# jinlinyi/PerspectiveFields

Hardware: NVIDIA H100
Metric: images/sec at 640x480 (Paramnet-360Cities-edina), H100 vs ref CPU (higher is better)
Workload: dtype f32 via 3x bf16 split MMA, fp32 accumulate

## Files before the change

perspectivefields_b200/csrc/gemm_tma.cuh:

```cuda
#pragma once
#include <cuda.h>

#include "tc_ptx.cuh"

namespace pf {

constexpr int MODE_GEMM = 0, MODE_HALO = 1;
constexpr int kTmaThreads = 384;
constexpr int kHaloBytes = 180 * 128;

struct TmaGemmParams {
  int M;
  int B, H, W;
  int Cin;
  int N, K;
  int a_c0, a_gc;
  int c_split, a2_c0;
  int groups;
  int b_row0;
  const float* bias; int bias_mode, bias_gstride;
  int act; const float* gamma;
  const float* res;  int ldr, r_coff, r_gcoff, res_relu;
  const float* res2; int ldr2, r2_coff, r2_gcoff;
  float* C; int ldc, c_coff, c_gcoff;
  __nv_bfloat16* Shi; __nv_bfloat16* Slo; int lds, s_coff, s_gcoff, split_relu;
  const float* pred_w; const float* pred_b; float* pred_out; int pred_nc, pred_mode;
  int phase4;
};

template <int BN, int MODE, int KB, bool PP = false, int NP = 3> struct TmaCfg {
  static_assert(KB == 32 || KB == 64, "KB");
  static_assert(BN % 32 == 0 && BN <= 256, "BN");
  static_assert(!PP || MODE == MODE_GEMM, "the ping-pong schedule is a GEMM-mode schedule");
  static_assert(NP == 1 || NP == 3, "NP");
  static constexpr int kPlanes = NP == 3 ? 2 : 1;
  static constexpr int kTileM = PP ? 64 : 128;
  static constexpr int kBPlane = BN * KB * 2;
  static constexpr int kAPlane = kTileM * KB * 2;
  static constexpr int kStage = (MODE == MODE_GEMM ? kPlanes * kAPlane : 0) + kPlanes * kBPlane;
  static constexpr int kABuf = kPlanes * kHtPlaneBytes;
  static constexpr int kAccPitch = 68;
  static constexpr int kAccStage = 2 * 64 * kAccPitch * 4;
  static constexpr int kBudget = 225 * 1024 - kAccStage - (MODE == MODE_HALO ? 2 * kABuf : 0);
  static constexpr int kStagesRaw = kBudget / kStage;
  static constexpr int kStages = kStagesRaw > 16 ? 16 : kStagesRaw;
  static constexpr int kSmemBytes = (MODE == MODE_HALO ? 2 * kABuf : 0) + kStages * kStage + kAccStage + 512 + 1024;
  static_assert(kStages >= 2, "ring too shallow");
  static_assert(kSmemBytes <= 227 * 1024, "shared memory per block");
};

__device__ __forceinline__ void mbar_expect_tx(uint32_t bar, uint32_t bytes) {
  asm volatile("mbarrier.arrive.expect_tx.shared::cta.b64 _, [%0], %1;\n" ::"r"(bar), "r"(bytes) : "memory");
}
__device__ __forceinline__ void tma_load_2d(uint32_t dst, const CUtensorMap* map, uint32_t bar, int c0, int c1) {
  asm volatile("cp.async.bulk.tensor.2d.shared::cluster.global.mbarrier::complete_tx::bytes [%0], [%1, {%3, %4}], [%2];\n"
               ::"r"(dst), "l"(reinterpret_cast<uint64_t>(map)), "r"(bar), "r"(c0), "r"(c1) : "memory");
}
__device__ __forceinline__ void tma_load_4d(uint32_t dst, const CUtensorMap* map, uint32_t bar, int c0, int c1, int c2, int c3) {
  asm volatile("cp.async.bulk.tensor.4d.shared::cluster.global.mbarrier::complete_tx::bytes [%0], [%1, {%3, %4, %5, %6}], [%2];\n"
               ::"r"(dst), "l"(reinterpret_cast<uint64_t>(map)), "r"(bar), "r"(c0), "r"(c1), "r"(c2), "r"(c3) : "memory");
}
__device__ __forceinline__ void tma_prefetch_desc(const CUtensorMap* map) {
  asm volatile("prefetch.tensormap [%0];\n" ::"l"(reinterpret_cast<uint64_t>(map)) : "memory");
}

struct TmaMaps {
  CUtensorMap a_hi, a_lo, a2_hi, a2_lo, b_hi, b_lo;
};

template <int BN, int MODE, int KB, bool PP = false, int NP = 3>
__global__ void __launch_bounds__(kTmaThreads, 1) gemm_tma_kernel(const __grid_constant__ TmaMaps maps, const TmaGemmParams p, int tiles_x, int tiles_y) {
  using Cfg = TmaCfg<BN, MODE, KB, PP, NP>;
  constexpr bool kLo = NP == 3;
  constexpr int NS = Cfg::kStages;
  constexpr int SPC = 9 * (64 / KB);
  constexpr int kConsumerWarps = PP ? 4 : 8;
  extern __shared__ unsigned char smem_dyn[];
  const uint32_t raw = smem_u32(smem_dyn);
  const uint32_t sbase = (raw + 1023u) & ~1023u;
  unsigned char* sm = smem_dyn + (sbase - raw);
  const uint32_t a_base = sbase;
  const uint32_t ring = sbase + (MODE == MODE_HALO ? 2 * Cfg::kABuf : 0);
  const uint32_t acc_base = ring + NS * Cfg::kStage;
  const uint32_t bars = acc_base + Cfg::kAccStage;
  auto full_b = [&](int s) { return bars + 8u * s; };
  auto empty_b = [&](int s) { return bars + 8u * (NS + s); };
  auto full_a = [&](int i) { return bars + 8u * (2 * NS + i); };
  auto empty_a = [&](int i) { return bars + 8u * (2 * NS + 2 + i); };
  auto order_b = [&](int w) { return bars + 8u * (2 * NS + 4 + w); };

  const int tid = threadIdx.x, lane = tid & 31, warp = tid >> 5;
  const int n_tiles = cdiv(p.N, BN);
  const int m_tiles = MODE == MODE_GEMM ? cdiv(p.M, Cfg::kTileM) : p.B * tiles_x * tiles_y;
  const int total_tiles = m_tiles * n_tiles * p.groups;
  const int nchunks = MODE == MODE_HALO ? p.Cin / 64 : 0;
  const int nk = MODE == MODE_GEMM ? p.K / KB : nchunks * SPC;
  const bool b_resident = MODE == MODE_HALO && nchunks == 1 && SPC <= NS;

  if (tid == 0) {
    tma_prefetch_desc(&maps.a_hi); tma_prefetch_desc(&maps.b_hi);
    if (kLo) { tma_prefetch_desc(&maps.a_lo); tma_prefetch_desc(&maps.b_lo); }
    for (int s = 0; s < NS; ++s) { mbar_init(full_b(s), 1); mbar_init(empty_b(s), kConsumerWarps); }
    for (int i = 0; i < 2; ++i) { mbar_init(full_a(i), 1); mbar_init(empty_a(i), kConsumerWarps); mbar_init(order_b(i), 4); }
    fence_mbar_init();
  }
  __syncthreads();
  pdl_wait();
  pdl_launch();

  auto decode = [&](int tile, int& mt, int& g, int& n0) {
    n0 = (tile % n_tiles) * BN;
    tile /= n_tiles;
    g = tile % p.groups;
    mt = tile / p.groups;
  };

  if (warp < 4) {
    asm volatile("setmaxnreg.dec.sync.aligned.u32 40;\n");
    if (warp == 0 && lane == 0) {
      int it = 0;
      for (int tile = blockIdx.x; tile < total_tiles; tile += gridDim.x) {
        int mt, g, n0;
        decode(tile, mt, g, n0);
        const int brow = p.b_row0 + g * p.N + n0;
        if (b_resident && it > 0) break;
        for (int kc = 0; kc < nk; ++kc, ++it) {
          const int s = it % NS;
          mbar_wait(empty_b(s), ((it / NS) & 1) ^ 1);
          mbar_expect_tx(full_b(s), Cfg::kStage);
          const uint32_t st = ring + s * Cfg::kStage;
          int kcol;
          if (MODE == MODE_GEMM) {
            kcol = kc * KB;
            tma_load_2d(st, &maps.a_hi, full_b(s), p.a_c0 + g * p.a_gc + kcol, mt * Cfg::kTileM);
            if (kLo) tma_load_2d(st + Cfg::kAPlane, &maps.a_lo, full_b(s), p.a_c0 + g * p.a_gc + kcol, mt * Cfg::kTileM);
          } else {
            const int c = kc / SPC, u = kc - c * SPC;
            kcol = KB == 32 ? (u >> 1) * p.Cin + c * 64 + (u & 1) * 32 : u * p.Cin + c * 64;
          }
          const uint32_t bdst = st + (MODE == MODE_GEMM ? Cfg::kPlanes * Cfg::kAPlane : 0);
          tma_load_2d(bdst, &maps.b_hi, full_b(s), kcol, brow);
          if (kLo) tma_load_2d(bdst + Cfg::kBPlane, &maps.b_lo, full_b(s), kcol, brow);
        }
      }
    } else if (MODE == MODE_HALO && warp == 1 && lane == 0) {
      int ita = 0;
      for (int tile = blockIdx.x; tile < total_tiles; tile += gridDim.x) {
        int mt, g, n0;
        decode(tile, mt, g, n0);
        const int tx = mt % tiles_x, ty = (mt / tiles_x) % tiles_y, bimg = mt / (tiles_x * tiles_y);
        for (int c = 0; c < nchunks; ++c, ++ita) {
          const int buf = ita & 1;
          mbar_wait(empty_a(buf), ((ita >> 1) & 1) ^ 1);
          mbar_expect_tx(full_a(buf), Cfg::kPlanes * kHaloBytes);
          const uint32_t dst = a_base + buf * Cfg::kABuf;
          const int ci = c * 64;
          if (p.c_split > 0 && ci >= p.c_split) {
            tma_load_4d(dst, &maps.a2_hi, full_a(buf), p.a2_c0 + ci - p.c_split, tx * kHtTileW - 1, ty * kHtTileH - 1, bimg);
            if (kLo) tma_load_4d(dst + kHtPlaneBytes, &maps.a2_lo, full_a(buf), p.a2_c0 + ci - p.c_split, tx * kHtTileW - 1, ty * kHtTileH - 1, bimg);
          } else {
            tma_load_4d(dst, &maps.a_hi, full_a(buf), p.a_c0 + g * p.a_gc + ci, tx * kHtTileW - 1, ty * kHtTileH - 1, bimg);
            if (kLo) tma_load_4d(dst + kHtPlaneBytes, &maps.a_lo, full_a(buf), p.a_c0 + g * p.a_gc + ci, tx * kHtTileW - 1, ty * kHtTileH - 1, bimg);
          }
        }
      }
    }
    return;
  }

  asm volatile("setmaxnreg.inc.sync.aligned.u32 232;\n");
  const int wg = (warp >> 2) - 1;
  const int wt = tid & 127;
  float* stage = reinterpret_cast<float*>(sm + (acc_base - sbase)) + wg * 64 * Cfg::kAccPitch;
  const int erow = wt & 63, eh = wt >> 6;
  const int r = PP ? erow : wg * 64 + erow;
  constexpr int kTileStep = PP ? 2 : 1;
  float acc[BN / 2];
  int it = 0, ita = 0;
  for (int tl = PP ? wg : 0, tile = blockIdx.x + tl * gridDim.x; tile < total_tiles; tile += kTileStep * gridDim.x, tl += kTileStep) {
    int mt, g, n0;
    decode(tile, mt, g, n0);
    if (PP) {
      it = tl * nk;
      if (tl > 0) mbar_wait(order_b(wg ^ 1), ((tl - 1) >> 1) & 1);
    }
    int prev_s = -1, prev_buf = -1;
    fence_regs(acc);
    for (int kc = 0; kc < nk; ++kc, ++it) {
      const int s = it % NS;
      uint32_t a_hi, a_lo;
      bool chunk_end = false;
      int buf = 0;
      if (MODE == MODE_HALO) {
        const int c = kc / SPC, u = kc - c * SPC;
        const int tap = KB == 32 ? (u >> 1) : u, ky = tap / 3, kx = tap - ky * 3;
        buf = ita & 1;
        if (u == 0) mbar_wait(full_a(buf), (ita >> 1) & 1);
        a_hi = a_base + buf * Cfg::kABuf + ((ky + 8 * wg) * kHtHaloW + kx) * 128 + (KB == 32 ? (u & 1) * 64 : 0);
        a_lo = a_hi + kHtPlaneBytes;
        chunk_end = u == SPC - 1;
      } else {
        a_hi = ring + s * Cfg::kStage + (PP ? 0 : wg * 64 * KB * 2);
        a_lo = a_hi + Cfg::kAPlane;
      }
      const int sb = b_resident ? kc : s;
      if (!b_resident || tl == 0) mbar_wait(full_b(sb), b_resident ? 0 : ((it / NS) & 1));
      const uint32_t b_hi = ring + sb * Cfg::kStage + (MODE == MODE_GEMM ? Cfg::kPlanes * Cfg::kAPlane : 0);
      const uint64_t dah = MODE == MODE_HALO ? ht_a_desc(a_hi) : wgmma_tile_desc<KB>(a_hi);
      const uint64_t dbh = wgmma_tile_desc<KB>(b_hi);
      wgmma_fence();
      if (kLo) {
        const uint64_t dal = MODE == MODE_HALO ? ht_a_desc(a_lo) : wgmma_tile_desc<KB>(a_lo);
        const uint64_t dbl = wgmma_tile_desc<KB>(b_hi + Cfg::kBPlane);
#pragma unroll
        for (int kk = 0; kk < KB / 16; ++kk) {
          const uint32_t first = (kc | kk) ? 1u : 0u;
          wgmma_bf16<BN>(acc, dal + 2 * kk, dbh + 2 * kk, first);
          wgmma_bf16<BN>(acc, dah + 2 * kk, dbl + 2 * kk, 1u);
          wgmma_bf16<BN>(acc, dah + 2 * kk, dbh + 2 * kk, 1u);
        }
      } else {
#pragma unroll
        for (int kk = 0; kk < KB / 16; ++kk) wgmma_bf16<BN>(acc, dah + 2 * kk, dbh + 2 * kk, (kc | kk) ? 1u : 0u);
      }
      wgmma_commit();
      wgmma_wait<1>();
      if (lane == 0 && prev_s >= 0) {
        if (!b_resident) mbar_arrive(empty_b(prev_s));
        if (MODE == MODE_HALO && prev_buf >= 0) mbar_arrive(empty_a(prev_buf));
      }
      prev_s = s;
      prev_buf = chunk_end ? buf : -1;
      if (MODE == MODE_HALO && chunk_end) ++ita;
    }
    if (PP && lane == 0) mbar_arrive(order_b(wg));
    wgmma_wait<0>();
    fence_regs(acc);
    if (lane == 0 && prev_s >= 0) {
      if (!b_resident) mbar_arrive(empty_b(prev_s));
      if (MODE == MODE_HALO && prev_buf >= 0) mbar_arrive(empty_a(prev_buf));
    }

    long long m;
    bool valid;
    int cls_off = 0;
    int bimg = 0, oy = 0, ox = 0, oy0 = 0, ox0 = 0;
    if (MODE == MODE_GEMM) {
      m = (long long)mt * Cfg::kTileM + r;
      valid = m < p.M;
    } else {
      const int tx = mt % tiles_x, ty = (mt / tiles_x) % tiles_y;
      bimg = mt / (tiles_x * tiles_y);
      oy0 = ty * kHtTileH; ox0 = tx * kHtTileW;
      oy = oy0 + (r >> 3); ox = ox0 + (r & 7);
      valid = oy < p.H && ox < p.W;
      m = ((long long)bimg * p.H + oy) * p.W + ox;
      if (p.bias_mode == 2) {
        const int ry = oy == 0 ? 0 : (oy == p.H - 1 ? 2 : 1);
        const int rx = ox == 0 ? 0 : (ox == p.W - 1 ? 2 : 1);
        cls_off = (ry * 3 + rx) * p.N;
      }
    }
    const float* __restrict__ bias = p.bias ? p.bias + (long long)g * p.bias_gstride : nullptr;
    auto stage_row = [&](int rr, long long& mr) -> bool {
      if (MODE == MODE_GEMM) {
        mr = (long long)mt * Cfg::kTileM + (PP ? 0 : wg * 64) + rr;
        return mr < p.M;
      }
      const int rt = wg * 64 + rr, py = oy0 + (rt >> 3), px = ox0 + (rt & 7);
      mr = ((long long)bimg * p.H + py) * p.W + px;
      return py < p.H && px < p.W;
    };
    const int frow = (wt >> 5) * 16 + (lane >> 2), fcol = 2 * (lane & 3);
#pragma unroll
    for (int rd = 0; rd < (BN + 63) / 64; ++rd) {
      named_bar_sync(1 + wg, 128);
#pragma unroll
      for (int jb = 0; jb < 8; ++jb) {
        const int cb = rd * 8 + jb;
        if (cb < BN / 8) {
          float* d0 = stage + frow * Cfg::kAccPitch + jb * 8 + fcol;
          *reinterpret_cast<float2*>(d0) = make_float2(acc[4 * cb], acc[4 * cb + 1]);
          *reinterpret_cast<float2*>(d0 + 8 * Cfg::kAccPitch) = make_float2(acc[4 * cb + 2], acc[4 * cb + 3]);
        }
      }
      named_bar_sync(1 + wg, 128);
      const int ch = 2 * rd + eh;
      const bool own = ch < BN / 32;
      const bool ph4 = MODE == MODE_HALO && BN == 128 && p.phase4;
      const bool staged_split = p.Shi && !ph4;
      const int nb = n0 + ch * 32;
      const bool chunk_ok = own && nb < p.N;
      const bool live = valid && chunk_ok;
      const float* srow = stage + erow * Cfg::kAccPitch + eh * 32;
      float o[32];
      if (own) {
#pragma unroll
        for (int j = 0; j < 32; j += 4) {
          const float4 t = *reinterpret_cast<const float4*>(srow + j);
          o[j] = t.x; o[j + 1] = t.y; o[j + 2] = t.z; o[j + 3] = t.w;
        }
      }
      if (live) {
        if (p.bias_mode) {
#pragma unroll
          for (int j = 0; j < 32; j += 4) {
            const float4 bv = __ldg(reinterpret_cast<const float4*>(bias + cls_off + nb + j));
            o[j] += bv.x; o[j + 1] += bv.y; o[j + 2] += bv.z; o[j + 3] += bv.w;
          }
        }
        if (p.act == 1) {
#pragma unroll
          for (int j = 0; j < 32; ++j) o[j] = fmaxf(o[j], 0.f);
        } else if (p.act == 2) {
#pragma unroll
          for (int j = 0; j < 32; ++j) o[j] = gelu_erf(o[j]);
        }
        if (p.gamma) {
#pragma unroll
          for (int j = 0; j < 32; j += 4) {
            const float4 gv = __ldg(reinterpret_cast<const float4*>(p.gamma + nb + j));
            o[j] *= gv.x; o[j + 1] *= gv.y; o[j + 2] *= gv.z; o[j + 3] *= gv.w;
          }
        }
      }
      auto stage_in = [&](const float* src, int ld, int coff) {
        named_bar_sync(1 + wg, 128);
        float4 v[8];
#pragma unroll
        for (int t = 0; t < 8; ++t) {
          const int i = wt + 128 * t, col = rd * 64 + (i & 15) * 4;
          long long mr;
          v[t] = make_float4(0.f, 0.f, 0.f, 0.f);
          if (col < BN && n0 + col < p.N && stage_row(i >> 4, mr)) v[t] = *reinterpret_cast<const float4*>(src + mr * ld + coff + n0 + col);
        }
#pragma unroll
        for (int t = 0; t < 8; ++t) {
          const int i = wt + 128 * t;
          *reinterpret_cast<float4*>(stage + (i >> 4) * Cfg::kAccPitch + (i & 15) * 4) = v[t];
        }
        named_bar_sync(1 + wg, 128);
      };
      if (p.res) {
        stage_in(p.res, p.ldr, p.r_coff + g * p.r_gcoff);
        if (live) {
#pragma unroll
          for (int j = 0; j < 32; j += 4) {
            float4 rv = *reinterpret_cast<const float4*>(srow + j);
            if (p.res_relu) { rv.x = fmaxf(rv.x, 0.f); rv.y = fmaxf(rv.y, 0.f); rv.z = fmaxf(rv.z, 0.f); rv.w = fmaxf(rv.w, 0.f); }
            o[j] += rv.x; o[j + 1] += rv.y; o[j + 2] += rv.z; o[j + 3] += rv.w;
          }
        }
      }
      if (p.res2) {
        stage_in(p.res2, p.ldr2, p.r2_coff + g * p.r2_gcoff);
        if (live) {
#pragma unroll
          for (int j = 0; j < 32; j += 4) {
            const float4 rv = *reinterpret_cast<const float4*>(srow + j);
            o[j] += rv.x; o[j + 1] += rv.y; o[j + 2] += rv.z; o[j + 3] += rv.w;
          }
        }
      }
      const long long mo = ph4 ? ((long long)bimg * 2 * p.H + 2 * oy + (ch >> 1)) * (2 * p.W) + 2 * ox + (ch & 1) : m;
      if (MODE == MODE_HALO && (BN == 32 || BN == 128) && p.pred_w && live) {
        float v0 = __ldg(p.pred_b), v1 = p.pred_nc > 1 ? __ldg(p.pred_b + 1) : 0.f;
#pragma unroll
        for (int j = 0; j < 32; j += 4) {
          const float4 w0 = __ldg(reinterpret_cast<const float4*>(p.pred_w + j));
          v0 = fmaf(o[j], w0.x, v0); v0 = fmaf(o[j + 1], w0.y, v0); v0 = fmaf(o[j + 2], w0.z, v0); v0 = fmaf(o[j + 3], w0.w, v0);
          if (p.pred_nc > 1) {
            const float4 w1 = __ldg(reinterpret_cast<const float4*>(p.pred_w + 32 + j));
            v1 = fmaf(o[j], w1.x, v1); v1 = fmaf(o[j + 1], w1.y, v1); v1 = fmaf(o[j + 2], w1.z, v1); v1 = fmaf(o[j + 3], w1.w, v1);
          }
        }
        const long long HWl = (long long)p.H * p.W * (ph4 ? 4 : 1);
        const long long bi = mo / HWl, pix = mo - bi * HWl;
        float* po = p.pred_out + bi * p.pred_nc * HWl + pix;
        if (p.pred_mode == 1) {
          const float nrm = fmaxf(sqrtf(v0 * v0 + v1 * v1), 1e-12f);
          po[0] = v0 / nrm; po[HWl] = v1 / nrm;
        } else {
          po[0] = fminf(fmaxf(v0, -1.f), 1.f);
        }
      }
      if (ph4 && chunk_ok && (p.C || p.Shi)) {
        const bool odd = lane & 1;
        const bool valid_p = __shfl_xor_sync(0xffffffffu, (int)valid, 1) != 0;
        const long long mo_p = mo + (odd ? -2 : 2);
        const long long moA = odd ? mo_p : mo, moB = odd ? mo : mo_p;
        const bool vA = odd ? valid_p : valid, vB = odd ? valid : valid_p;
        if (p.C) {
          float* cA = p.C + moA * p.ldc + p.c_coff + g * p.c_gcoff + (odd ? 4 : 0);
          float* cB = p.C + moB * p.ldc + p.c_coff + g * p.c_gcoff + (odd ? 4 : 0);
#pragma unroll
          for (int t = 0; t < 4; ++t) {
            float k[4], rr[4];
#pragma unroll
            for (int e = 0; e < 4; ++e) {
              k[e] = odd ? o[8 * t + 4 + e] : o[8 * t + e];
              rr[e] = __shfl_xor_sync(0xffffffffu, odd ? o[8 * t + e] : o[8 * t + 4 + e], 1);
            }
            if (vA) *reinterpret_cast<float4*>(cA + 8 * t) = odd ? make_float4(rr[0], rr[1], rr[2], rr[3]) : make_float4(k[0], k[1], k[2], k[3]);
            if (vB) *reinterpret_cast<float4*>(cB + 8 * t) = odd ? make_float4(k[0], k[1], k[2], k[3]) : make_float4(rr[0], rr[1], rr[2], rr[3]);
          }
        }
        if (p.Shi) {
          const long long sA = moA * p.lds + p.s_coff + g * p.s_gcoff + (odd ? 8 : 0);
          const long long sB = moB * p.lds + p.s_coff + g * p.s_gcoff + (odd ? 8 : 0);
#pragma unroll
          for (int t = 0; t < 2; ++t) {
            float k[8], rr[8];
#pragma unroll
            for (int e = 0; e < 8; ++e) {
              const float mine = odd ? o[16 * t + 8 + e] : o[16 * t + e], give = odd ? o[16 * t + e] : o[16 * t + 8 + e];
              k[e] = p.split_relu ? fmaxf(mine, 0.f) : mine;
              rr[e] = __shfl_xor_sync(0xffffffffu, p.split_relu ? fmaxf(give, 0.f) : give, 1);
            }
            uint4 kh, kl, rh, rl;
            split_bf16x2(k[0], k[1], kh.x, kl.x); split_bf16x2(k[2], k[3], kh.y, kl.y);
            split_bf16x2(k[4], k[5], kh.z, kl.z); split_bf16x2(k[6], k[7], kh.w, kl.w);
            split_bf16x2(rr[0], rr[1], rh.x, rl.x); split_bf16x2(rr[2], rr[3], rh.y, rl.y);
            split_bf16x2(rr[4], rr[5], rh.z, rl.z); split_bf16x2(rr[6], rr[7], rh.w, rl.w);
            if (vA) {
              *reinterpret_cast<uint4*>(p.Shi + sA + 16 * t) = odd ? rh : kh;
              *reinterpret_cast<uint4*>(p.Slo + sA + 16 * t) = odd ? rl : kl;
            }
            if (vB) {
              *reinterpret_cast<uint4*>(p.Shi + sB + 16 * t) = odd ? kh : rh;
              *reinterpret_cast<uint4*>(p.Slo + sB + 16 * t) = odd ? kl : rl;
            }
          }
        }
      }
      if (p.C && !ph4) {
        named_bar_sync(1 + wg, 128);
        if (own) {
          float* drow = stage + erow * Cfg::kAccPitch + eh * 32;
#pragma unroll
          for (int j = 0; j < 32; j += 4) *reinterpret_cast<float4*>(drow + j) = make_float4(o[j], o[j + 1], o[j + 2], o[j + 3]);
        }
        named_bar_sync(1 + wg, 128);
        float* cbase = p.C + p.c_coff + g * p.c_gcoff + n0;
#pragma unroll
        for (int t = 0; t < 8; ++t) {
          const int i = wt + 128 * t, col = rd * 64 + (i & 15) * 4;
          long long mr;
          if (col < BN && n0 + col < p.N && stage_row(i >> 4, mr))
            *reinterpret_cast<float4*>(cbase + mr * p.ldc + col) = *reinterpret_cast<const float4*>(stage + (i >> 4) * Cfg::kAccPitch + (i & 15) * 4);
        }
      }
      if (staged_split) {
        named_bar_sync(1 + wg, 128);
        unsigned char* sS = reinterpret_cast<unsigned char*>(stage);
        if (own) {
#pragma unroll
          for (int t = 0; t < 4; ++t) {
            uint4 h, l;
            float k[8];
#pragma unroll
            for (int e = 0; e < 8; ++e) k[e] = p.split_relu ? fmaxf(o[8 * t + e], 0.f) : o[8 * t + e];
            split_bf16x2(k[0], k[1], h.x, l.x); split_bf16x2(k[2], k[3], h.y, l.y);
            split_bf16x2(k[4], k[5], h.z, l.z); split_bf16x2(k[6], k[7], h.w, l.w);
            const int off = erow * 128 + (((eh * 4 + t) ^ (erow & 7)) << 4);
            *reinterpret_cast<uint4*>(sS + off) = h;
            *reinterpret_cast<uint4*>(sS + 64 * 128 + off) = l;
          }
        }
        named_bar_sync(1 + wg, 128);
#pragma unroll
        for (int i = wt; i < 2 * 64 * 8; i += 128) {
          const int lo_plane = i >> 9, rr = (i >> 3) & 63, pc = i & 7;
          const int col = rd * 64 + pc * 8;
          long long mr;
          if (col >= BN || n0 + col >= p.N || !stage_row(rr, mr)) continue;
          const uint4 v = *reinterpret_cast<const uint4*>(sS + lo_plane * 64 * 128 + rr * 128 + ((pc ^ (rr & 7)) << 4));
          *reinterpret_cast<uint4*>((lo_plane ? p.Slo : p.Shi) + mr * p.lds + p.s_coff + g * p.s_gcoff + n0 + col) = v;
        }
      }
    }
  }
}

}
```

perspectivefields_b200/csrc/tc_ptx.cuh:

```cuda
#pragma once
#include "common.cuh"

namespace pf {

constexpr int kHtTileH = 16, kHtTileW = 8;
constexpr int kHtHaloW = kHtTileW + 2, kHtHaloH = kHtTileH + 2;
constexpr int kHtHaloPix = kHtHaloW * kHtHaloH;
constexpr int kHtPlaneBytes = 23 * 1024;

__device__ __forceinline__ void mbar_init(uint32_t bar, uint32_t count) {
  asm volatile("mbarrier.init.shared::cta.b64 [%0], %1;\n" ::"r"(bar), "r"(count) : "memory");
}
__device__ __forceinline__ void mbar_arrive(uint32_t bar) {
  asm volatile("mbarrier.arrive.shared::cta.b64 _, [%0];\n" ::"r"(bar) : "memory");
}
__device__ __forceinline__ uint32_t mbar_try_wait(uint32_t bar, uint32_t parity) {
  uint32_t ok;
  asm volatile("{\n\t.reg .pred p;\n\tmbarrier.try_wait.parity.shared::cta.b64 p, [%1], %2;\n\tselp.u32 %0, 1, 0, p;\n\t}\n"
               : "=r"(ok) : "r"(bar), "r"(parity) : "memory");
  return ok;
}
__device__ __forceinline__ void mbar_wait(uint32_t bar, uint32_t parity) {
  if (mbar_try_wait(bar, parity)) return;
  const long long t0 = clock64();
  while (!mbar_try_wait(bar, parity)) {
    if (clock64() - t0 > 4000000000LL) __trap();
  }
}
__device__ __forceinline__ void fence_mbar_init() { asm volatile("fence.mbarrier_init.release.cluster;\n" ::: "memory"); }
__device__ __forceinline__ void named_bar_sync(int id, int count) { asm volatile("bar.sync %0, %1;\n" ::"r"(id), "r"(count) : "memory"); }

__device__ __forceinline__ void wgmma_fence() { asm volatile("wgmma.fence.sync.aligned;\n" ::: "memory"); }
__device__ __forceinline__ void wgmma_commit() { asm volatile("wgmma.commit_group.sync.aligned;\n" ::: "memory"); }
template <int N>
__device__ __forceinline__ void wgmma_wait() { asm volatile("wgmma.wait_group.sync.aligned %0;\n" ::"n"(N) : "memory"); }
template <int R>
__device__ __forceinline__ void fence_regs(float (&d)[R]) {
#pragma unroll
  for (int i = 0; i < R; ++i) asm volatile("" : "+f"(d[i])::"memory");
}

#define PF_R8(i) "+f"(d[i]), "+f"(d[i + 1]), "+f"(d[i + 2]), "+f"(d[i + 3]), "+f"(d[i + 4]), "+f"(d[i + 5]), "+f"(d[i + 6]), "+f"(d[i + 7])
template <int N> struct Wgmma;
template <> struct Wgmma<32> {
  static __device__ __forceinline__ void mma(float* d, uint64_t adesc, uint64_t bdesc, uint32_t scale_d) {
    asm volatile(
      "{\n\t.reg .pred p;\n\tsetp.ne.b32 p, %18, 0;\n\t"
      "wgmma.mma_async.sync.aligned.m64n32k16.f32.bf16.bf16 {"
      "%0,%1,%2,%3,%4,%5,%6,%7,%8,%9,%10,%11,%12,%13,%14,%15"
      "}, %16, %17, p, 1, 1, 0, 0;\n\t}\n"
      : PF_R8(0), PF_R8(8)
      : "l"(adesc), "l"(bdesc), "r"(scale_d));
  }
};
template <> struct Wgmma<64> {
  static __device__ __forceinline__ void mma(float* d, uint64_t adesc, uint64_t bdesc, uint32_t scale_d) {
    asm volatile(
      "{\n\t.reg .pred p;\n\tsetp.ne.b32 p, %34, 0;\n\t"
      "wgmma.mma_async.sync.aligned.m64n64k16.f32.bf16.bf16 {"
      "%0,%1,%2,%3,%4,%5,%6,%7,%8,%9,%10,%11,%12,%13,%14,%15,%16,%17,%18,%19,%20,%21,%22,%23,%24,%25,%26,%27,%28,%29,%30,%31"
      "}, %32, %33, p, 1, 1, 0, 0;\n\t}\n"
      : PF_R8(0), PF_R8(8), PF_R8(16), PF_R8(24)
      : "l"(adesc), "l"(bdesc), "r"(scale_d));
  }
};
template <> struct Wgmma<96> {
  static __device__ __forceinline__ void mma(float* d, uint64_t adesc, uint64_t bdesc, uint32_t scale_d) {
    asm volatile(
      "{\n\t.reg .pred p;\n\tsetp.ne.b32 p, %50, 0;\n\t"
      "wgmma.mma_async.sync.aligned.m64n96k16.f32.bf16.bf16 {"
      "%0,%1,%2,%3,%4,%5,%6,%7,%8,%9,%10,%11,%12,%13,%14,%15,%16,%17,%18,%19,%20,%21,%22,%23,%24,%25,%26,%27,%28,%29,%30,%31,"
      "%32,%33,%34,%35,%36,%37,%38,%39,%40,%41,%42,%43,%44,%45,%46,%47"
      "}, %48, %49, p, 1, 1, 0, 0;\n\t}\n"
      : PF_R8(0), PF_R8(8), PF_R8(16), PF_R8(24), PF_R8(32), PF_R8(40)
      : "l"(adesc), "l"(bdesc), "r"(scale_d));
  }
};
template <> struct Wgmma<128> {
  static __device__ __forceinline__ void mma(float* d, uint64_t adesc, uint64_t bdesc, uint32_t scale_d) {
    asm volatile(
      "{\n\t.reg .pred p;\n\tsetp.ne.b32 p, %66, 0;\n\t"
      "wgmma.mma_async.sync.aligned.m64n128k16.f32.bf16.bf16 {"
      "%0,%1,%2,%3,%4,%5,%6,%7,%8,%9,%10,%11,%12,%13,%14,%15,%16,%17,%18,%19,%20,%21,%22,%23,%24,%25,%26,%27,%28,%29,%30,%31,"
      "%32,%33,%34,%35,%36,%37,%38,%39,%40,%41,%42,%43,%44,%45,%46,%47,%48,%49,%50,%51,%52,%53,%54,%55,%56,%57,%58,%59,%60,%61,%62,%63"
      "}, %64, %65, p, 1, 1, 0, 0;\n\t}\n"
      : PF_R8(0), PF_R8(8), PF_R8(16), PF_R8(24), PF_R8(32), PF_R8(40), PF_R8(48), PF_R8(56)
      : "l"(adesc), "l"(bdesc), "r"(scale_d));
  }
};
template <> struct Wgmma<160> {
  static __device__ __forceinline__ void mma(float* d, uint64_t adesc, uint64_t bdesc, uint32_t scale_d) {
    asm volatile(
      "{\n\t.reg .pred p;\n\tsetp.ne.b32 p, %82, 0;\n\t"
      "wgmma.mma_async.sync.aligned.m64n160k16.f32.bf16.bf16 {"
      "%0,%1,%2,%3,%4,%5,%6,%7,%8,%9,%10,%11,%12,%13,%14,%15,%16,%17,%18,%19,%20,%21,%22,%23,%24,%25,%26,%27,%28,%29,%30,%31,"
      "%32,%33,%34,%35,%36,%37,%38,%39,%40,%41,%42,%43,%44,%45,%46,%47,%48,%49,%50,%51,%52,%53,%54,%55,%56,%57,%58,%59,%60,%61,%62,%63,"
      "%64,%65,%66,%67,%68,%69,%70,%71,%72,%73,%74,%75,%76,%77,%78,%79"
      "}, %80, %81, p, 1, 1, 0, 0;\n\t}\n"
      : PF_R8(0), PF_R8(8), PF_R8(16), PF_R8(24), PF_R8(32), PF_R8(40), PF_R8(48), PF_R8(56), PF_R8(64), PF_R8(72)
      : "l"(adesc), "l"(bdesc), "r"(scale_d));
  }
};
template <> struct Wgmma<192> {
  static __device__ __forceinline__ void mma(float* d, uint64_t adesc, uint64_t bdesc, uint32_t scale_d) {
    asm volatile(
      "{\n\t.reg .pred p;\n\tsetp.ne.b32 p, %98, 0;\n\t"
      "wgmma.mma_async.sync.aligned.m64n192k16.f32.bf16.bf16 {"
      "%0,%1,%2,%3,%4,%5,%6,%7,%8,%9,%10,%11,%12,%13,%14,%15,%16,%17,%18,%19,%20,%21,%22,%23,%24,%25,%26,%27,%28,%29,%30,%31,"
      "%32,%33,%34,%35,%36,%37,%38,%39,%40,%41,%42,%43,%44,%45,%46,%47,%48,%49,%50,%51,%52,%53,%54,%55,%56,%57,%58,%59,%60,%61,%62,%63,"
      "%64,%65,%66,%67,%68,%69,%70,%71,%72,%73,%74,%75,%76,%77,%78,%79,%80,%81,%82,%83,%84,%85,%86,%87,%88,%89,%90,%91,%92,%93,%94,%95"
      "}, %96, %97, p, 1, 1, 0, 0;\n\t}\n"
      : PF_R8(0), PF_R8(8), PF_R8(16), PF_R8(24), PF_R8(32), PF_R8(40), PF_R8(48), PF_R8(56), PF_R8(64), PF_R8(72), PF_R8(80), PF_R8(88)
      : "l"(adesc), "l"(bdesc), "r"(scale_d));
  }
};
template <> struct Wgmma<224> {
  static __device__ __forceinline__ void mma(float* d, uint64_t adesc, uint64_t bdesc, uint32_t scale_d) {
    asm volatile(
      "{\n\t.reg .pred p;\n\tsetp.ne.b32 p, %114, 0;\n\t"
      "wgmma.mma_async.sync.aligned.m64n224k16.f32.bf16.bf16 {"
      "%0,%1,%2,%3,%4,%5,%6,%7,%8,%9,%10,%11,%12,%13,%14,%15,%16,%17,%18,%19,%20,%21,%22,%23,%24,%25,%26,%27,%28,%29,%30,%31,"
      "%32,%33,%34,%35,%36,%37,%38,%39,%40,%41,%42,%43,%44,%45,%46,%47,%48,%49,%50,%51,%52,%53,%54,%55,%56,%57,%58,%59,%60,%61,%62,%63,"
      "%64,%65,%66,%67,%68,%69,%70,%71,%72,%73,%74,%75,%76,%77,%78,%79,%80,%81,%82,%83,%84,%85,%86,%87,%88,%89,%90,%91,%92,%93,%94,%95,"
      "%96,%97,%98,%99,%100,%101,%102,%103,%104,%105,%106,%107,%108,%109,%110,%111"
      "}, %112, %113, p, 1, 1, 0, 0;\n\t}\n"
      : PF_R8(0), PF_R8(8), PF_R8(16), PF_R8(24), PF_R8(32), PF_R8(40), PF_R8(48), PF_R8(56), PF_R8(64), PF_R8(72), PF_R8(80), PF_R8(88), PF_R8(96), PF_R8(104)
      : "l"(adesc), "l"(bdesc), "r"(scale_d));
  }
};
template <> struct Wgmma<256> {
  static __device__ __forceinline__ void mma(float* d, uint64_t adesc, uint64_t bdesc, uint32_t scale_d) {
    asm volatile(
      "{\n\t.reg .pred p;\n\tsetp.ne.b32 p, %130, 0;\n\t"
      "wgmma.mma_async.sync.aligned.m64n256k16.f32.bf16.bf16 {"
      "%0,%1,%2,%3,%4,%5,%6,%7,%8,%9,%10,%11,%12,%13,%14,%15,%16,%17,%18,%19,%20,%21,%22,%23,%24,%25,%26,%27,%28,%29,%30,%31,"
      "%32,%33,%34,%35,%36,%37,%38,%39,%40,%41,%42,%43,%44,%45,%46,%47,%48,%49,%50,%51,%52,%53,%54,%55,%56,%57,%58,%59,%60,%61,%62,%63,"
      "%64,%65,%66,%67,%68,%69,%70,%71,%72,%73,%74,%75,%76,%77,%78,%79,%80,%81,%82,%83,%84,%85,%86,%87,%88,%89,%90,%91,%92,%93,%94,%95,"
      "%96,%97,%98,%99,%100,%101,%102,%103,%104,%105,%106,%107,%108,%109,%110,%111,%112,%113,%114,%115,%116,%117,%118,%119,%120,%121,%122,%123,%124,%125,%126,%127"
      "}, %128, %129, p, 1, 1, 0, 0;\n\t}\n"
      : PF_R8(0), PF_R8(8), PF_R8(16), PF_R8(24), PF_R8(32), PF_R8(40), PF_R8(48), PF_R8(56), PF_R8(64), PF_R8(72), PF_R8(80), PF_R8(88), PF_R8(96), PF_R8(104), PF_R8(112), PF_R8(120)
      : "l"(adesc), "l"(bdesc), "r"(scale_d));
  }
};
#undef PF_R8
template <int N>
__device__ __forceinline__ void wgmma_bf16(float* d, uint64_t adesc, uint64_t bdesc, uint32_t scale_d) { Wgmma<N>::mma(d, adesc, bdesc, scale_d); }

template <int KB>
__device__ __forceinline__ uint64_t wgmma_tile_desc(uint32_t smem_addr) {
  constexpr uint64_t sbo = KB == 32 ? 512 : 1024, layout = KB == 32 ? 2 : 1;
  return (uint64_t)((smem_addr >> 4) & 0x3FFFu) | ((uint64_t)1 << 16) | ((sbo >> 4) << 32) | (layout << 62);
}
__device__ __forceinline__ uint64_t ht_a_desc(uint32_t smem_addr) {
  return (uint64_t)((smem_addr >> 4) & 0x3FFFu) | ((uint64_t)1 << 16) | ((uint64_t)((kHtHaloW * 128) >> 4) << 32) |
         ((uint64_t)1 << 62);
}

}
```

Measured before the change: 807.6.

## Prefetch residual via cp.async into lent halo buffer during epilogue

In halo-mode 3-plane GEMMs that carry a residual, the consumer holds back the last A halo buffer instead of releasing it, and reuses it as a staging slot. Residual tiles are fetched with cp.async one round ahead, so global loads overlap the accumulator staging and epilogue math, replacing the synchronous stage_in loads. The buffer is released after the epilogue with an async-proxy fence. This costs a longer hold on one producer buffer, which can stall the TMA producer, plus extra barrier syncs.

```diff
diff --git a/perspectivefields_b200/csrc/gemm_tma.cuh b/perspectivefields_b200/csrc/gemm_tma.cuh
--- a/perspectivefields_b200/csrc/gemm_tma.cuh
+++ b/perspectivefields_b200/csrc/gemm_tma.cuh
@@ -175,6 +175,9 @@
   const int erow = wt & 63, eh = wt >> 6;
   const int r = PP ? erow : wg * 64 + erow;
   constexpr int kTileStep = PP ? 2 : 1;
+  constexpr int kResSlot = 64 * Cfg::kAccPitch * 4;
+  static_assert(MODE != MODE_HALO || NP != 3 || 2 * kResSlot <= Cfg::kABuf, "lent halo buffer");
+  const bool lend = MODE == MODE_HALO && NP == 3 && p.res != nullptr;
   float acc[BN / 2];
   int it = 0, ita = 0;
   for (int tl = PP ? wg : 0, tile = blockIdx.x + tl * gridDim.x; tile < total_tiles; tile += kTileStep * gridDim.x, tl += kTileStep) {
@@ -238,7 +241,7 @@
     fence_regs(acc);
     if (lane == 0 && prev_s >= 0) {
       if (!b_resident) mbar_arrive(empty_b(prev_s));
-      if (MODE == MODE_HALO && prev_buf >= 0) mbar_arrive(empty_a(prev_buf));
+      if (MODE == MODE_HALO && prev_buf >= 0 && !lend) mbar_arrive(empty_a(prev_buf));
     }
 
     long long m;
@@ -271,6 +274,24 @@
       mr = ((long long)bimg * p.H + py) * p.W + px;
       return py < p.H && px < p.W;
     };
+    const uint32_t xres = a_base + prev_buf * Cfg::kABuf + wg * kResSlot;
+    auto copy_round = [&](uint32_t dst, const float* src, int ld, int coff, int rd) {
+      const int col = rd * 64 + (wt & 15) * 4, px = ox0 + (wt >> 4), py0 = oy0 + 8 * wg;
+      const bool cok = col < BN && n0 + col < p.N && px < p.W;
+      const float* sp = src + (((long long)bimg * p.H + py0) * p.W + px) * ld + coff + n0 + col;
+      const long long step = (long long)p.W * ld;
+      dst += ((wt >> 4) * Cfg::kAccPitch + (wt & 15) * 4) * 4;
+#pragma unroll 1
+      for (int t = 0; t < 8; ++t, sp += step, dst += 8 * Cfg::kAccPitch * 4) {
+        const bool ok = cok && py0 + t < p.H;
+        cp_async16(dst, ok ? sp : src, ok);
+      }
+    };
+    if (lend) {
+      named_bar_sync(3, 256);
+      copy_round(xres, p.res, p.ldr, p.r_coff + g * p.r_gcoff, 0);
+      cp_async_commit();
+    }
     const int frow = (wt >> 5) * 16 + (lane >> 2), fcol = 2 * (lane & 3);
 #pragma unroll
     for (int rd = 0; rd < (BN + 63) / 64; ++rd) {
@@ -341,7 +362,37 @@
         }
         named_bar_sync(1 + wg, 128);
       };
-      if (p.res) {
+      if (lend) {
+        named_bar_sync(1 + wg, 128);
+        if (p.res2) copy_round(smem_u32(stage), p.res2, p.ldr2, p.r2_coff + g * p.r2_gcoff, rd);
+        cp_async_commit();
+        cp_async_wait<1>();
+        named_bar_sync(1 + wg, 128);
+        if (live) {
+          const float* xrow = reinterpret_cast<const float*>(sm + (xres - sbase)) + erow * Cfg::kAccPitch + eh * 32;
+#pragma unroll
+          for (int j = 0; j < 32; j += 4) {
+            float4 rv = *reinterpret_cast<const float4*>(xrow + j);
+            if (p.res_relu) { rv.x = fmaxf(rv.x, 0.f); rv.y = fmaxf(rv.y, 0.f); rv.z = fmaxf(rv.z, 0.f); rv.w = fmaxf(rv.w, 0.f); }
+            o[j] += rv.x; o[j + 1] += rv.y; o[j + 2] += rv.z; o[j + 3] += rv.w;
+          }
+        }
+        if (rd + 1 < (BN + 63) / 64) {
+          named_bar_sync(1 + wg, 128);
+          copy_round(xres, p.res, p.ldr, p.r_coff + g * p.r_gcoff, rd + 1);
+        }
+        cp_async_commit();
+        cp_async_wait<1>();
+        named_bar_sync(1 + wg, 128);
+        if (p.res2 && live) {
+#pragma unroll
+          for (int j = 0; j < 32; j += 4) {
+            const float4 rv = *reinterpret_cast<const float4*>(srow + j);
+            o[j] += rv.x; o[j + 1] += rv.y; o[j + 2] += rv.z; o[j + 3] += rv.w;
+          }
+        }
+      }
+      if (p.res && !lend) {
         stage_in(p.res, p.ldr, p.r_coff + g * p.r_gcoff);
         if (live) {
 #pragma unroll
@@ -352,7 +403,7 @@
           }
         }
       }
-      if (p.res2) {
+      if (p.res2 && !lend) {
         stage_in(p.res2, p.ldr2, p.r2_coff + g * p.r2_gcoff);
         if (live) {
 #pragma unroll
@@ -479,6 +530,11 @@
         }
       }
     }
+    if (lend) {
+      fence_proxy_async_smem();
+      __syncwarp();
+      if (lane == 0) mbar_arrive(empty_a(prev_buf));
+    }
   }
 }
 
diff --git a/perspectivefields_b200/csrc/tc_ptx.cuh b/perspectivefields_b200/csrc/tc_ptx.cuh
--- a/perspectivefields_b200/csrc/tc_ptx.cuh
+++ b/perspectivefields_b200/csrc/tc_ptx.cuh
@@ -28,6 +28,7 @@
   }
 }
 __device__ __forceinline__ void fence_mbar_init() { asm volatile("fence.mbarrier_init.release.cluster;\n" ::: "memory"); }
+__device__ __forceinline__ void fence_proxy_async_smem() { asm volatile("fence.proxy.async.shared::cta;\n" ::: "memory"); }
 __device__ __forceinline__ void named_bar_sync(int id, int count) { asm volatile("bar.sync %0, %1;\n" ::"r"(id), "r"(count) : "memory"); }
 
 __device__ __forceinline__ void wgmma_fence() { asm volatile("wgmma.fence.sync.aligned;\n" ::: "memory"); }
```

New measurement: 817.9, median of 6. 1.3% higher.
